# meudnaes/VoronoiRT

Hardware: AMD Instinct MI355X
Metric: formal-solve cell-updates/sec (higher is better)
Workload: dtype f64

## Files before the change

include/voronoirt.h:

```cpp
#ifndef VORONOIRT_H
#define VORONOIRT_H

#include <stdint.h>

#ifdef __cplusplus
extern "C" {
#endif

#define VRT_OK 0
#define VRT_EINVAL (-1)
#define VRT_EGRID (-2)
#define VRT_ENODEVICE (-3)
#define VRT_ENOMEM (-4)
#define VRT_EIO (-5)

typedef struct vrt_grid vrt_grid;
typedef struct vrt_plan vrt_plan;

#define VRT_ALPHA_SITE 0
#define VRT_ALPHA_SITE_LAM 1
#define VRT_ALPHA_ANGLE_SITE_LAM 2
#define VRT_ALPHA_ANGLE_NATIVE 3
#define VRT_ALPHA_SITE_LAM_NATIVE 4

// ... 80 lines not shown
                                     double *max_rel_change, void *stream);
int vrt_rates_populations_native_dev_f32(vrt_plan *p, int64_t nlam, const double *lambda, const int64_t blocks[6],
                                         const float *dJ_up, const float *dJ_down, const double *planck2,
                                         double lambda0, double c0, const double *d_doppler_width, const double *d_gamma,
                                         double sigma_bb_const, const double *sigma_bf1, const double *sigma_bf2,
                                         const double *d_temperature, const double *d_lte_populations, double hc_over_kB,
                                         double pref_ij, double pref_ji, const double *d_C, const double *d_atom_density,
                                         double *d_R, double *d_populations, void *stream);

int vrt_plan_execute_dev_f32(vrt_plan *p, int64_t nlam, int64_t ld, const float *dS,
                             const float *dalpha, int alpha_mode, const float *dI0_up,
                             const float *dI0_down, const double *weights_host, float *dJ,
                             float *dI_out, void *stream);
int vrt_plan_last_sweep_timing(const vrt_plan *p, double *ms, int64_t *launches);
int vrt_plan_patch_layout(const vrt_plan *p, int64_t *out);
int vrt_plan_check(vrt_plan *p);
int vrt_plan_last_path(const vrt_plan *p);
int vrt_plan_set_option(vrt_plan *p, const char *name, const char *value);
int vrt_grid_set_option(vrt_grid *g, const char *name, const char *value);

typedef struct vrt_schedule vrt_schedule;
int vrt_schedule_build(const vrt_grid *g, int dir, const int64_t *up, int n_sweeps, vrt_schedule **out);
int64_t vrt_schedule_num_nodes(const vrt_schedule *s);
int64_t vrt_schedule_num_levels(const vrt_schedule *s);
int vrt_schedule_get(const vrt_schedule *s, int64_t *site, int32_t *zflags, int64_t *level_off);
void vrt_schedule_destroy(vrt_schedule *s);
int vrt_layer_schedule(const vrt_grid *g, int dir, const int64_t *up, int n_sweeps, uint32_t *vis,
                       int32_t *nlev, int64_t *n_visits);
int vrt_layer_sorted_slots(const vrt_grid *g, int dir, const uint32_t *vis, int64_t *store, int64_t *self);

// ... 240 lines not shown
```

voronoirt_amd/_lib.py:

```python
from __future__ import annotations

import ctypes
import os

HERE = os.path.dirname(os.path.abspath(__file__))
LIB_PATH = os.path.join(HERE, "libvrt_hip.so")
if os.environ.get("VRT_LIB_PATH"):
    LIB_PATH = os.environ["VRT_LIB_PATH"]

c_i64 = ctypes.c_int64
c_dbl = ctypes.c_double
p_i64 = ctypes.POINTER(ctypes.c_int64)
p_i32 = ctypes.POINTER(ctypes.c_int32)
p_dbl = ctypes.POINTER(ctypes.c_double)
p_int = ctypes.POINTER(ctypes.c_int)
vp = ctypes.c_void_p

VRT_OK, VRT_EINVAL, VRT_EGRID, VRT_ENODEVICE, VRT_ENOMEM, VRT_EIO = 0, -1, -2, -3, -4, -5
ALPHA_SITE, ALPHA_SITE_LAM, ALPHA_ANGLE_SITE_LAM, ALPHA_ANGLE_NATIVE, ALPHA_SITE_LAM_NATIVE = 0, 1, 2, 3, 4
METRIC_EUCLIDEAN, METRIC_PERIODIC_XY = 0, 1
RASTER_NEAREST, RASTER_INV_DIST2 = 1, 2

class LineCaseStruct(ctypes.Structure):
    _fields_ = [("nlam", c_i64), ("lambda_", p_dbl), ("blocks", c_i64 * 6), ("lambda0", c_dbl), ("c0", c_dbl),
# ... 80 lines not shown
    "vrt_multi_set_shard": (ctypes.c_int, [vp, ctypes.c_char_p]),
    "vrt_multi_last_shard": (ctypes.c_int, [vp]),
    "vrt_multi_uses_rccl": (ctypes.c_int, [vp]),
    "vrt_multi_destroy": (None, [vp]),
    "vrt_multi_execute_line": (ctypes.c_int, [vp, c_i64, c_i64, p_dbl, c_dbl, c_dbl, p_dbl, p_dbl, p_dbl, p_dbl, p_dbl, p_dbl,
                                              p_dbl, p_dbl, p_dbl, p_dbl]),
    "vrt_multi_lambda_create": (ctypes.c_int, [vp, ctypes.POINTER(LineCaseStruct), p_dbl, ctypes.POINTER(vp)]),
    "vrt_multi_lambda_iterate": (ctypes.c_int, [vp, p_dbl]),
    "vrt_multi_lambda_get": (ctypes.c_int, [vp, p_dbl, p_dbl, p_dbl, p_dbl, p_dbl]),
    "vrt_multi_lambda_destroy": (None, [vp]),
    "vrt_rates_populations_dev": (ctypes.c_int, [vp, c_i64, c_i64, p_dbl, p_i64, vp, p_dbl, c_dbl, c_dbl, vp, vp,
                                                 c_dbl, p_dbl, p_dbl, vp, vp, c_dbl, c_dbl, c_dbl, vp, vp, vp,
                                                 vp, vp]),
    "vrt_plan_last_sweep_timing": (ctypes.c_int, [vp, p_dbl, p_i64]),
    "vrt_plan_patch_layout": (ctypes.c_int, [vp, p_i64]),
    "vrt_plan_last_path": (ctypes.c_int, [vp]),
    "vrt_plan_set_option": (ctypes.c_int, [vp, ctypes.c_char_p, ctypes.c_char_p]),
    "vrt_grid_set_option": (ctypes.c_int, [vp, ctypes.c_char_p, ctypes.c_char_p]),
    "vrt_schedule_build": (ctypes.c_int, [vp, ctypes.c_int, p_i64, ctypes.c_int,
                                          ctypes.POINTER(vp)]),
    "vrt_schedule_num_nodes": (c_i64, [vp]),
    "vrt_schedule_num_levels": (c_i64, [vp]),
    "vrt_schedule_get": (ctypes.c_int, [vp, p_i64, p_i32, p_i64]),
    "vrt_schedule_destroy": (None, [vp]),
    "vrt_layer_schedule": (ctypes.c_int, [vp, ctypes.c_int, p_i64, ctypes.c_int,
                                          ctypes.POINTER(ctypes.c_uint32), p_i32, p_i64]),
    "vrt_layer_sorted_slots": (ctypes.c_int, [vp, ctypes.c_int, ctypes.POINTER(ctypes.c_uint32), p_i64, p_i64]),
    "vrt_patch_schedule_build": (ctypes.c_int, [vp, ctypes.c_int, p_i64, ctypes.c_int, ctypes.c_int, ctypes.c_int,
                                                ctypes.POINTER(vp), p_i64]),
    "vrt_patch_schedule_get": (ctypes.c_int, [vp, p_i32, p_i32, p_i32, p_i32, p_i64, p_i32,
# ... 127 lines not shown
```

voronoirt_amd/csrc/vrt_api.cpp:

```cpp
#include <algorithm>
#include <atomic>
#include <chrono>
#include <cmath>
#include <cstdio>
#include <cstdlib>
#include <cstring>
#include <memory>
#include <new>
#include <thread>

#include "vrt_internal.h"

namespace vrt {

static thread_local std::string g_err;

void set_error(const std::string &msg) { g_err = msg; }
int fail(int code, const std::string &msg)
{
    g_err = msg;
    return code;
}

int check_source(const double *S, int64_t count)
// ... 14 lines not shown
{
    if (S)
        if (int rc = check_source(S, n * nlam)) return rc;
    if (populations)
        for (int64_t i = 0; i < 3 * n; i++)
            if (!std::isfinite(populations[i]) || !(populations[i] >= 0.0))
                return fail(VRT_EINVAL, "the populations must be finite and >= 0 everywhere");
    return VRT_OK;
}

void tuning_from_env(Tuning &t)
{
    static const char *names[] = {"VRT_PATH", "VRT_STEP_K", "VRT_STEP_SINGLE", "VRT_STEP_PAIRS", "VRT_STEP_XCD",
                                  "VRT_STEP_STREAMS", "VRT_STEP_LEVEL_MAP", "VRT_STEP_GROUP_DIR", "VRT_TILE_WIDE",
                                  "VRT_TILE_PRE", "VRT_PATCH_K", "VRT_PATCH_NT", "VRT_PATCH_OWN",
                                  "VRT_PATCH_Q", "VRT_PATCH_TARGET", "VRT_PATCH_SPLIT", "VRT_PAIR_BLOCK", "VRT_PATCH_QUAD", "VRT_PATCH_LEAN", "VRT_PATCH_CHAIN", "VRT_CHAIN_PAIRS", "VRT_CHAIN_SPIN", "VRT_CHAIN_DATAFLAG", "VRT_CHAIN_STATIC", "VRT_LAMBDA_NATIVE", "VRT_DEBUG_FLAGS", "VRT_DEBUG_SKIP_LEVELS",
                                  "VRT_TILE_DEBUG"};
    for (const char *nm : names) {
        const char *e = std::getenv(nm);
        if (e && *e && tuning_set(t, nm, e, false) != VRT_OK) {
            static std::mutex mu;
            static std::vector<std::string> said;
            std::lock_guard<std::mutex> lock(mu);
            if (std::find(said.begin(), said.end(), std::string(nm)) == said.end()) {
                said.push_back(nm);
                std::fprintf(stderr, "[libvrt_hip] ignoring %s=%s: %s\n", nm, e, g_err.c_str());
            }
        }
    }
}

// ... 7 lines not shown
            if (v == paths[i]) { t.path = i; return VRT_OK; }
        if (v.empty()) { t.path = 0; return VRT_OK; }
        return fail(VRT_EINVAL, "VRT_PATH must be auto, levels, tiles, steps or patches");
    }
    char *end = nullptr;
    const long x = std::strtol(value, &end, 10);
    if (end == value || *end != 0) return fail(VRT_EINVAL, "option " + nm + " needs an integer value");
    struct { const char *name; int *field; long lo, hi; bool creation_only; } tab[] = {
        {"VRT_STEP_K", &t.step_K, 0, 18, false}, {"VRT_STEP_SINGLE", &t.step_single, 0, 1, false},
        {"VRT_STEP_PAIRS", &t.step_pairs, 0, 64, false}, {"VRT_STEP_XCD", &t.step_xcd, 0, 2, false},
        {"VRT_STEP_STREAMS", &t.step_streams, 1, 4, false}, {"VRT_STEP_LEVEL_MAP", &t.step_level_map, 0, 1, false},
        {"VRT_STEP_GROUP_DIR", &t.step_group_dir, 0, 1, false}, {"VRT_TILE_WIDE", &t.tile_wide, 0, 1, false},
        {"VRT_TILE_PRE", &t.tile_pre, 0, 1, false},
        {"VRT_PATCH_K", &t.patch_K, 1, 8, true}, {"VRT_PATCH_NT", &t.patch_NT, 64, 1024, true},
        {"VRT_PATCH_OWN", &t.patch_own, 0, 65535, true}, {"VRT_PATCH_Q", &t.patch_Q, 1, 4, false},
        {"VRT_PATCH_TARGET", &t.patch_target, 0, 1 << 20, false}, {"VRT_PATCH_SPLIT", &t.patch_split, 0, 4096, false}, {"VRT_PAIR_BLOCK", &t.pair_block, 1, 16, true},
        {"VRT_PATCH_QUAD", &t.patch_quad, 0, 1, true}, {"VRT_PATCH_LEAN", &t.patch_lean, 0, 1, false},
        {"VRT_PATCH_CHAIN", &t.patch_chain, 0, 2, false}, {"VRT_CHAIN_PAIRS", &t.chain_pairs, 1, 256, false},
        {"VRT_CHAIN_SPIN", &t.chain_spin, 1, 1 << 20, false}, {"VRT_CHAIN_DATAFLAG", &t.chain_dataflag, 0, 2, false},
        {"VRT_LAMBDA_NATIVE", &t.lambda_native, 0, 1, false}, {"VRT_CHAIN_STATIC", &t.chain_static, 0, 1, false}, {"VRT_DEBUG_FLAGS", &t.debug_flags, 0, 1 << 20, false},
        {"VRT_DEBUG_SKIP_LEVELS", &t.debug_skip_levels, 0, 1, false}, {"VRT_TILE_DEBUG", &t.tile_debug, 0, 1, false},
    };
    for (auto &o : tab)
        if (nm == o.name) {
            if (o.creation_only && created)
                return fail(VRT_EINVAL, "option " + nm + " shapes what plan creation builds: preset it in the environment");
            if (x < o.lo || x > o.hi) return fail(VRT_EINVAL, "option " + nm + " out of range");
            *o.field = (int)x;
            return VRT_OK;
        }
    return fail(VRT_EINVAL, "unknown option " + nm);
// ... 1185 lines not shown
        fewest = INT64_MAX;
        for (int a = 0; a < p->A; a++)
            for (int layer = 2; layer <= maxL; layer++) {
                const int32_t *first = p->h_patch_first.data() + (size_t)a * (size_t)(maxL + 2);
                fewest = std::min<int64_t>(fewest, first[layer + 1] - first[layer]);
            }
        if (fewest == INT64_MAX) fewest = 0;
    }
    out[0] = p->patch_ok ? p->n_patches : 0;
    out[1] = fewest;
    out[2] = p->patch_work_off.empty() ? 0 : p->patch_work_off.back();
    out[3] = p->patch_work_padding;
    return VRT_OK;
}

int vrt_plan_last_sweep_timing(const vrt_plan *p, double *ms, int64_t *launches)
{
    if (!p) return fail(VRT_EINVAL, "NULL plan");
    if (!p->ev_valid) return fail(VRT_EINVAL, "no execute has run on this plan yet");
    return guarded([&] {
        VRT_HIP_TRY(hipEventSynchronize(p->ev1));
        float t = 0.f;
        VRT_HIP_TRY(hipEventElapsedTime(&t, p->ev0, p->ev1));
        if (ms) *ms = (double)t;
        if (launches) *launches = p->last_launches;
        return patch_chain_check(const_cast<vrt_plan *>(p));
    });
}

int vrt_plan_last_path(const vrt_plan *p) { return p ? p->last_path : 0; }
// ... 302 lines not shown
```

voronoirt_amd/csrc/vrt_internal.h:

```cpp
#pragma once

#include <hip/hip_runtime.h>

#include <algorithm>
#include <cstdint>
#include <memory>
#include <mutex>
#include <new>
#include <string>
#include <thread>
#include <vector>

#include "voronoirt.h"

namespace vrt {

void set_error(const std::string &msg);
int fail(int code, const std::string &msg);

int check_source(const double *S, int64_t count);
int check_state_pointers(const void *session, const double *S, const double *populations);
int check_state(int64_t n, int64_t nlam, const double *S, const double *populations);

#define VRT_HIP_TRY(expr)                                                                  \
// ... 211 lines not shown
    int step_group_dir = 1;
    int tile_wide = 1;
    int tile_pre = 1;
    int patch_K = 1, patch_NT = 512;
    int patch_own = 0;
    int patch_Q = 1;
    int pair_block = 1;
    int patch_quad = 1;
    int patch_lean = 1;
    int patch_chain = 2;
    int chain_pairs = 9;
    int chain_spin = 2048;
    int chain_dataflag = 2;
    int patch_split = 0;
    int patch_target = 0;
    int chain_static = 1;
    int lambda_native = 1;
    int debug_flags = 0, debug_skip_levels = 0, tile_debug = 0;
};
void tuning_from_env(Tuning &t);
int tuning_set(Tuning &t, const char *name, const char *value, bool created);

struct ExecArgs {
    int64_t nlam = 0, ld = 0;
    const void *S = nullptr;
    const void *S_nat[2] = {nullptr, nullptr};
    const void *alpha = nullptr;
    int alpha_mode = 0;
    const void *I0[2] = {nullptr, nullptr};
    const double *weights = nullptr;
// ... 153 lines not shown
    int chain_npair = -1, chain_lgB = -1, chain_nsplit = -1, chain_reduce = -1;
    int64_t chain_items = 0;
    struct ChainSet {
        int npair = -1, lgB = -1, nsplit = -1, reduce = -1;
        vrt::DevBuf<int4> items;
        vrt::DevBuf<int32_t> deps;
        int q_off[9] = {0, 0, 0, 0, 0, 0, 0, 0, 0};
        int64_t n_items = 0;
    };
    std::vector<ChainSet> chain_cache;
    uint32_t chain_epoch = 0;
    vrt::DevBuf<int4> d_patch_work;
    std::vector<int64_t> patch_work_off;
    int patch_work_groups = 0;
    int64_t patch_work_padding = 0;
    vrt::Stream step_stream[4];
    vrt::Event step_fork, step_join[4];
    int last_path = 0;
    vrt::Event ev0, ev1;
    bool ev_valid = false;
    std::vector<vrt::CopyLane> copy_lanes;
    vrt::Event copy_done;
    int64_t last_launches = 0;
    std::mutex mu;
};

namespace vrt {

struct PlanDelete { void operator()(vrt_plan *p) const { vrt_plan_destroy(p); } };
using PlanPtr = std::unique_ptr<vrt_plan, PlanDelete>;
// ... 136 lines not shown
int plane_from_native_f32(vrt_plan *p, int dir_index, int64_t nlam, int64_t ld, const float *din, float *dout, hipStream_t st);
int J_from_native_f32(vrt_plan *p, int64_t nlam, int64_t ld, const float *dJ_up, const float *dJ_down, float *dJ, hipStream_t st);
int planes_to_native(vrt_plan *p, int64_t nlam, int64_t ld, const double *din, double *out_up, double *out_down, hipStream_t st);
int plane_from_native(vrt_plan *p, int dir_index, int64_t nlam, int64_t ld, const double *din, double *dout, hipStream_t st);
int J_from_native(vrt_plan *p, int64_t nlam, int64_t ld, const double *dJ_up, const double *dJ_down, double *dJ, hipStream_t st);
int execute_layers(vrt_plan *p, const ExecArgs &x, int path);
int64_t steps_max_layer(bool f32);

struct TileArgs;
struct PatchReduce;
bool patch_shape_exists(int K, int Q, int NT);
int launch_patch_entries(vrt_plan *p, int a, int64_t first, int64_t count);
int ensure_patch_work(vrt_plan *p, int G, const std::vector<int32_t> &group_angles, const std::vector<int> &group_off);
int launch_patch_layer(vrt_plan *p, const TileArgs &ta, int npair, int layer, int group, int Q, hipStream_t st,
                       bool f32, const PatchReduce *reduce);
bool patch_chain_possible(const vrt_plan *p, int npair, bool f32);
bool patch_chain_dataflag(const vrt_plan *p, int npair, bool f32);
int launch_patch_chain(vrt_plan *p, const TileArgs &ta, int npair, hipStream_t st, bool f32, const PatchReduce *reduce,
                       bool dataflag, bool ctrl_zeroed = false);
int chain_ctrl_words();
int patch_chain_check(vrt_plan *p);

struct NgRange {
    int64_t dense = 0, tail = 0, tstride = 1;
};
struct NgState {
    int order = 0, start = 0, period = 0;
    DevBuf<double> hist[3];
    unsigned have = 0;
    DevBuf<double> d_ws;
// ... 12 lines not shown
```

voronoirt_amd/csrc/vrt_layers.hip:

```cpp
#include <hip/hip_runtime.h>

#include <algorithm>
#include <cmath>
#include <cstdio>
#include <cstdlib>
#include <cstring>

#include "vrt_device.h"
#include "vrt_internal.h"

#include "vrt_layout_kernels.h"
#include "vrt_step_kernels.h"
#include "vrt_tile_kernels.h"

namespace vrt {

static int build_task_map(vrt_plan *p, int nlam, hipStream_t st)
{
    const int A = p->A;
    if (p->task_map_nlam == nlam && p->d_task_map) return VRT_OK;
    const int ntask = A * nlam;
    struct Group { int a, l0, l1; double cost; };
    std::vector<Group> groups;
    const int halves = nlam >= 2 ? 2 : 1;
// ... 649 lines not shown
            if (upto <= reduced_upto[d]) continue;
            red.lo[k] = (int)reduced_upto[d];
            red.hi[k] = (int)upto;
            red.Jd[k] = J_planes(p, x, d);
            red.count[k] = 0;
            for (int a = 0; a < A; a++)
                if ((p->dir_of_active[(size_t)a] > 0) == (d == 0)) red.angles[k][red.count[k]++] = a;
            reduced_upto[d] = upto;
            k++;
        }
        return k > 0;
    };
    const int Lmax = deepest_layer(r);
    if ((rc = fork_streams(p, st, G))) return rc;
    r.launches = 0;
    for (int layer = 2; layer <= Lmax; layer++)
        for (int gi = 0; gi < G; gi++) {
            hipStream_t sg = gi == 0 ? st : p->step_stream[gi];
            if (p->step_group_off[gi + 1] == p->step_group_off[gi]) continue;
            int Q = p->tune.patch_Q;
            if (!patch_shape_exists(p->patch_K, Q, p->patch_NT) || (npair % Q != 0 && npair < 2 * Q)) Q = 1;
            PatchReduce red;
            const bool have_red = make_reduce(gi, layer - 1, false, red);
            if ((rc = launch_patch_layer(p, r.ta, npair, layer, gi, Q, sg, kF32, have_red ? &red : nullptr))) return rc;
            r.launches += 1;
        }
    for (int gi = 0; gi < G; gi++) {
        PatchReduce red;
        if (!make_reduce(gi, 0, true, red)) continue;
        if ((rc = launch_patch_layer(p, r.ta, npair, p->tile_max_layers + 1, gi, 1, gi == 0 ? st : p->step_stream[gi], kF32, &red)))
// ... 139 lines not shown
```

voronoirt_amd/csrc/vrt_patch.hip:

```cpp
#include <hip/hip_runtime.h>

#include <algorithm>
#include <cmath>
#include <cstdio>
#include <cstdlib>
#include <cstring>
#include <type_traits>

#include "vrt_device.h"
#include "vrt_internal.h"

namespace vrt {

enum : int {
    kDiagNoLevels = 1, kDiagCentreGathers = 2, kDiagNoWeights = 4, kDiagNoStores = 8, kDiagNoGatherI = 16, kDiagNoGatherAlpha = 32,
    kDiagNoGatherS = 64, kDiagNoReduce = 128, kDiagNoWait = 256, kDiagPlainLoadI = 512, kDiagPlainStoreI = 1024, kDiagNoPairLoop = 2048,
    kDiagDirectTable = 4096,
};
__host__ __device__ __forceinline__ constexpr bool diag(int dbg, int flag) { return kDiag && (dbg & flag) != 0; }

struct PatchArgs {
    TileArgs ta;
    int npair;
    int layer;
    int ngrp;
    int nrow;
    int nsplit, Q;
    int sbase, srem;
    int lgB;
    int stride;
    int cap;
    int quad;
    int lean;
    int dbg_ent0, dbg_ent_stride, dbg_ent_last;
    int dbg;
    PatchReduce red;
    const int4 *wrec;
    const int32_t *e_pos, *e_u1, *e_u2;
    const uint32_t *e_vis, *e_loc;
    const double *e_w1, *e_w2, *e_r1, *e_r2;
};

__global__ void __launch_bounds__(256)
k_patch_entries(int64_t count, const int32_t *__restrict__ e_pos, const int32_t *__restrict__ t_u1,
                const int32_t *__restrict__ t_u2, const double *__restrict__ t_w1, const double *__restrict__ t_w2,
                const double *__restrict__ t_r1, const double *__restrict__ t_r2, int32_t *__restrict__ e_u1,
                int32_t *__restrict__ e_u2, double *__restrict__ e_w1, double *__restrict__ e_w2,
                double *__restrict__ e_r1, double *__restrict__ e_r2)
{
    const int64_t e = (int64_t)blockIdx.x * blockDim.x + threadIdx.x;
// ... 32 lines not shown
    const int nstep = (nblock + pa.Q - 1) / pa.Q;
    pa.sbase = nstep / pa.nsplit;
    pa.srem = nstep - pa.sbase * pa.nsplit;
}
__host__ __device__ __forceinline__ void split_blocks(const PatchArgs &pa, int split, int nblock, int &b0, int &b1)
{
    const int base = pa.sbase, rem = pa.srem;
    const int s0 = split * base + (split < rem ? split : rem), s1 = s0 + base + (split < rem ? 1 : 0);
    b0 = s0 * pa.Q;
    b1 = nblock < s1 * pa.Q ? nblock : s1 * pa.Q;
}

#ifndef VRT_REDUCE_LAST
#define VRT_REDUCE_LAST 1
#endif
__device__ __forceinline__ int reduce_block_index(const PatchArgs &pa)
{
    const int rows = (int)gridDim.y - pa.nrow;
    const int y = VRT_REDUCE_LAST ? (int)blockIdx.y - pa.nrow : ((int)blockIdx.y < rows ? (int)blockIdx.y : -1);
    return y < 0 ? -1 : y * (int)gridDim.x + (int)blockIdx.x;
}
__device__ __forceinline__ int patch_row(const PatchArgs &pa)
{
    return VRT_REDUCE_LAST ? (int)blockIdx.y : (int)blockIdx.y - ((int)gridDim.y - pa.nrow);
}
template <typename T, int NT>
__device__ __forceinline__ void patch_reduce_role(const PatchArgs &pa)
{
    typedef typename Pair<T>::type T2;
    const TileArgs &ta = pa.ta;
    const int tid = threadIdx.x;
    int b = reduce_block_index(pa), r = 0;
    if (b >= pa.red.nblk[0]) { b -= pa.red.nblk[0]; r = 1; }
    if (b >= pa.red.nblk[r]) return;
    if (diag(pa.dbg, kDiagNoReduce)) return;
    const int len = pa.red.hi[r] - pa.red.lo[r];
    const int per = NT * pa.red.ppb;
    const int nblock = pair_block_count(pa.npair, pa.lgB);
    int k0 = 0, lw = 0;
    for (int k = 0; k < nblock; k++) {
// ... 48 lines not shown
}

#ifdef VRT_PATCH_WPE
#define VRT_WPE_ATTR __attribute__((amdgpu_waves_per_eu(VRT_PATCH_WPE, VRT_PATCH_WPE)))
#else
#define VRT_WPE_ATTR
#endif
template <typename T, int AM, int K, int Q, int NT>
__global__ void __launch_bounds__(NT) VRT_WPE_ATTR
k_patch_solve(PatchArgs pa)
{
    typedef typename Pair<T>::type T2;
    extern __shared__ __attribute__((aligned(16))) double2 ptile[];
    const TileArgs &ta = pa.ta;
    const int tid = threadIdx.x;
    if (reduce_block_index(pa) >= 0) {
        patch_reduce_role<T, NT>(pa);
        return;
    }
    const int x = (int)blockIdx.x & 7, grp = (int)blockIdx.x >> 3, sj = patch_row(pa);
    const int4 rec = pa.wrec[2 * (sj * 8 + x)], rec2 = pa.wrec[2 * (sj * 8 + x) + 1];
    if (rec.y <= 0) return;
    const int sib = grp & ((1 << pa.lgB) - 1);
    const int nblock = pair_block_count(pa.npair, pa.lgB);
    int b0, b1;
    split_blocks(pa, grp >> pa.lgB, nblock, b0, b1);
    if (b0 >= b1) return;
    {
        int k0, lw;
        pair_block_of(b0, pa.npair, pa.lgB, k0, lw);
        if (sib >= (1 << lw)) return;
    }
    const int ent_off = rec.x, n_ent = rec.y, own_lo = rec.z, own_cnt = rec.w;
    const int dbg = kDiag ? pa.dbg : 0;
    const int nlev = diag(dbg, kDiagNoLevels) ? 0 : rec2.x, a = rec2.y & 0xFFFF;
    const int d = rec2.y >> 16;
    const int lo = rec2.z, hi = rec2.w;
    const int64_t n = ta.n;
    const int stride = pa.stride;

    double *s_w1 = reinterpret_cast<double *>(ptile + Q * stride);
    double *s_w2 = s_w1 + pa.cap, *s_r1 = s_w2 + pa.cap, *s_r2 = s_r1 + pa.cap;
    int *s_pos = reinterpret_cast<int *>(s_r2 + pa.cap);
    int *s_u1 = s_pos + pa.cap, *s_u2 = s_u1 + pa.cap;
    uint32_t *s_vis = reinterpret_cast<uint32_t *>(s_u2 + pa.cap), *s_loc = s_vis + pa.cap;
#pragma unroll
    for (int k = 0; k < K; k++) {
// ... 119 lines not shown
            }
        }
    }
}


typedef int vrt_i32x8 __attribute__((ext_vector_type(8)));
typedef const __attribute__((address_space(4))) vrt_i32x8 WorkRec;
static_assert(2 * sizeof(int4) == 32 && sizeof(vrt_i32x8) == 32, "a work-list slot is two int4: 32 bytes, 32-byte aligned");
struct PatchItem {
    int sib, b0, b1;
    int ent_off, n_ent, own_lo, own_cnt, nlev, a, d, lo, hi;
};
__device__ __forceinline__ bool patch_item(const PatchArgs &pa, int lgS, PatchItem &it)
{
    const int x = (int)blockIdx.x & 7, grp = (int)blockIdx.x >> 3, sj = patch_row(pa);
    const vrt_i32x8 r8 = *((const WorkRec *)(uintptr_t)pa.wrec + (sj * 8 + x));
    const int4 rec = make_int4(r8[0], r8[1], r8[2], r8[3]), rec2 = make_int4(r8[4], r8[5], r8[6], r8[7]);
    if (rec.y <= 0) return false;
    it.sib = grp & ((1 << lgS) - 1);
    split_blocks(pa, grp >> lgS, pair_block_count(pa.npair, pa.lgB), it.b0, it.b1);
    if (it.b0 >= it.b1) return false;
    it.ent_off = rec.x; it.n_ent = rec.y; it.own_lo = rec.z; it.own_cnt = rec.w;
    it.nlev = rec2.x; it.a = rec2.y & 0xFFFF;
    it.d = rec2.y >> 16;
    it.lo = rec2.z;
    it.hi = rec2.w;
    return true;
}
template <int CAP>
struct EntryTable {
    double *w1, *w2, *r1, *r2;
    int *pos, *u1, *u2;
    uint32_t *vis, *loc;
    __device__ __forceinline__ EntryTable(double2 *tiles, int planes)
    {
// ... 378 lines not shown
            } else {
                T2 *I = reinterpret_cast<T2 *>(pa.I) + (size_t)it.a * pa.npair * (size_t)n + qb;
                *reinterpret_cast<T2 *>(reinterpret_cast<char *>(I) + ((unsigned)(it.own_lo + tid) << sh)) = from_d2<T>(ptile[tid]);
            }
        }
        __syncthreads();
    }
}

template <typename T, int AM, int NT>
__global__ void __launch_bounds__(NT) VRT_LEAN_ATTR
k_patch_lean(PatchArgs pa)
{
    extern __shared__ __attribute__((aligned(16))) double2 ptile[];
    const int tid = threadIdx.x;
    if (reduce_block_index(pa) >= 0) {
        patch_reduce_role<T, NT>(pa);
        return;
    }
    const double e2 = exp2_table_load();
    typename EntryTable<NT>::Regs early{};
    if (diag(pa.dbg, kDiagDirectTable))
        early = EntryTable<NT>::load(pa, min(pa.dbg_ent0 + (patch_row(pa) * 8 + ((int)blockIdx.x & 7)) * pa.dbg_ent_stride + tid, pa.dbg_ent_last));
    PatchItem it;
    if (!patch_item(pa, pa.lgB, it)) return;
    if (diag(pa.dbg, kDiagNoPairLoop)) it.b1 = it.b0;
    const EntryTable<NT> tab(ptile, 1);
    if (tid == 0) ptile[it.n_ent] = make_double2(0.0, 0.0);
    if (diag(pa.dbg, kDiagDirectTable)) tab.store(early, it, tid);
    else tab.park(pa, it, tid);
    exp2_table_store(e2);
    __syncthreads();
    lean_pairs<T, AM, NT, 0>(pair_io<AM>(pa, it.d), it, tab, ptile);
}


template <int AM, int NT, bool CHAIN>
__device__ __forceinline__ void quad_pairs(const PairIO &pa, const PatchItem &it, const EntryTable<NT> &tab,
                                           double2 *ptile)
{
// ... 109 lines not shown
            }
        }
        __syncthreads();
    }
}

#ifndef VRT_QUAD_ATTR
#define VRT_QUAD_ATTR __attribute__((amdgpu_waves_per_eu(6, 6)))
#endif
template <int AM, int NT>
__global__ void __launch_bounds__(NT) VRT_QUAD_ATTR
k_patch_quad(PatchArgs pa)
{
    extern __shared__ __attribute__((aligned(16))) double2 ptile[];
    const int tid = threadIdx.x;
    if (reduce_block_index(pa) >= 0) {
        patch_reduce_role<float, NT>(pa);
        return;
    }
    const double e2 = exp2_table_load();
    PatchItem it;
    if (!patch_item(pa, pa.lgB - 1, it)) return;
    const EntryTable<NT> tab(ptile, 2);
    if (tid == 0) {
        ptile[it.n_ent] = make_double2(0.0, 0.0);
        ptile[NT + 1 + it.n_ent] = make_double2(0.0, 0.0);
    }
    tab.park(pa, it, tid);
    exp2_table_store(e2);
    __syncthreads();
    quad_pairs<AM, NT, false>(pair_io<AM>(pa, it.d), it, tab, ptile);
}


struct ChainDev {
    TileArgs ta;
    int npair, nsplit, cap;
// ... 388 lines not shown
            const int s_min = (int)std::min<int64_t>(steps_all, std::max<int64_t>(1, (512 + items - 1) / items));
            double dmin = 1e300;
            for (int c = steps_all; c >= 1; c--) {
                const int sc = (steps_all + c - 1) / c;
                if (sc >= s_min) dmin = std::min(dmin, std::fabs(std::log((double)items * sc / T)));
            }
            nsplit = s_min;
            for (int c = steps_all; c >= 1; c--) {
                const int sc = (steps_all + c - 1) / c;
                if (sc >= s_min && std::fabs(std::log((double)items * sc / T)) <= dmin + 0.03) nsplit = sc;
            }
        }
        pa.nsplit = nsplit;
        pa.ngrp = nsplit << lgS;
    }
    set_split(pa, pair_block_count(npair, pa.lgB));
    pa.stride = p->patch_cap + 1;
    pa.cap = p->patch_cap;
    pa.dbg = kDiag ? p->tune.debug_flags : 0;
    {
        const int64_t slots = std::max<int64_t>(1, p->patch_work_off.back());
        pa.dbg_ent_stride = (int)std::max<int64_t>(1, p->n_patch_entries / slots);
        pa.dbg_ent0 = (int)(w0 * pa.dbg_ent_stride);
        pa.dbg_ent_last = (int)std::max<int64_t>(0, p->n_patch_entries - 1);
    }
    pa.wrec = p->d_patch_work + 2 * w0;
    pa.e_pos = p->e_pos; pa.e_u1 = p->e_u1; pa.e_u2 = p->e_u2;
    pa.e_vis = p->e_vis; pa.e_loc = p->e_loc;
    pa.e_w1 = p->e_w1; pa.e_w2 = p->e_w2; pa.e_r1 = p->e_r1; pa.e_r2 = p->e_r2;
    pa.nrow = (int)((w1 - w0) / 8);
    int64_t gx = 8 * (int64_t)pa.ngrp;
    if (pa.nrow == 0) gx = std::max<int64_t>(gx, (((int64_t)pa.red.nred + 65534) / 65535 + 7) / 8 * 8);
    const int64_t gy = pa.nrow + (pa.red.nred + gx - 1) / gx;
    if (gy > 65535 || gx > INT32_MAX)
        return fail(VRT_EINVAL, "a layer of this size needs more than 65535 rows of patch and reduction blocks in one launch");
    const dim3 grid((unsigned)gx, (unsigned)gy);
    const size_t lds = (size_t)(pa.quad ? 2 : Q) * (size_t)pa.stride * sizeof(double2) + (size_t)pa.cap * (4 * sizeof(double) + 5 * sizeof(int32_t));
    const int rc = f32 ? launch_mode<float>(ta.alpha_mode, p->patch_K, Q, p->patch_NT, grid, lds, st, pa)
                       : launch_mode<double>(ta.alpha_mode, p->patch_K, Q, p->patch_NT, grid, lds, st, pa);
    return rc;
}

bool patch_chain_possible(const vrt_plan *p, int npair, bool f32)
{
    if (!p->patch_ok || p->tune.patch_chain == 0 || p->patch_K != 1 || p->patch_NT != 512) return false;
    const int lgB = native_lg(p, f32);
    const bool quad = f32 && lgB >= 1 && p->tune.patch_quad != 0 && (npair & 1) == 0;
    if (lgB - (quad ? 1 : 0) != 0) return false;
    if (!f32 && p->tune.patch_lean == 0) return false;
    if (p->tile_max_layers >= 65535 || p->A > 63) return false;
    if (p->tune.patch_chain == 1) return true;
    if (f32) return false;
    const double per_layer = (double)p->n_patches / (double)std::max(1, p->tile_max_layers);
    return per_layer * (double)pair_block_count(npair, lgB) <= 1400.0;
}
// ... 296 lines not shown
```

Before: 89.46 billion.

## Reorder patch-layer grid so split index maps to grid rows, add diagnostic timeline

```diff
diff --git a/include/voronoirt.h b/include/voronoirt.h
--- a/include/voronoirt.h
+++ b/include/voronoirt.h
@@ -118,6 +118,8 @@
                              float *dI_out, void *stream);
 int vrt_plan_last_sweep_timing(const vrt_plan *p, double *ms, int64_t *launches);
 int vrt_plan_patch_layout(const vrt_plan *p, int64_t *out);
+int vrt_patch_dispatch_map(int order, int nrow, int nsplit, int lg_siblings, int64_t nred, int steps, int64_t *dims, int32_t *blocks);
+int vrt_plan_patch_timeline(vrt_plan *p, int64_t cap_launches, int64_t cap_blocks, int64_t *launches, uint64_t *stamps, int64_t *counts);
 int vrt_plan_check(vrt_plan *p);
 int vrt_plan_last_path(const vrt_plan *p);
 int vrt_plan_set_option(vrt_plan *p, const char *name, const char *value);
diff --git a/voronoirt_amd/_lib.py b/voronoirt_amd/_lib.py
--- a/voronoirt_amd/_lib.py
+++ b/voronoirt_amd/_lib.py
@@ -118,6 +118,8 @@
                                                  vp, vp]),
     "vrt_plan_last_sweep_timing": (ctypes.c_int, [vp, p_dbl, p_i64]),
     "vrt_plan_patch_layout": (ctypes.c_int, [vp, p_i64]),
+    "vrt_patch_dispatch_map": (ctypes.c_int, [ctypes.c_int, ctypes.c_int, ctypes.c_int, ctypes.c_int, c_i64, ctypes.c_int, p_i64, p_i32]),
+    "vrt_plan_patch_timeline": (ctypes.c_int, [vp, c_i64, c_i64, p_i64, ctypes.POINTER(ctypes.c_uint64), p_i64]),
     "vrt_plan_last_path": (ctypes.c_int, [vp]),
     "vrt_plan_set_option": (ctypes.c_int, [vp, ctypes.c_char_p, ctypes.c_char_p]),
     "vrt_grid_set_option": (ctypes.c_int, [vp, ctypes.c_char_p, ctypes.c_char_p]),
diff --git a/voronoirt_amd/csrc/vrt_api.cpp b/voronoirt_amd/csrc/vrt_api.cpp
--- a/voronoirt_amd/csrc/vrt_api.cpp
+++ b/voronoirt_amd/csrc/vrt_api.cpp
@@ -52,7 +52,7 @@
     static const char *names[] = {"VRT_PATH", "VRT_STEP_K", "VRT_STEP_SINGLE", "VRT_STEP_PAIRS", "VRT_STEP_XCD",
                                   "VRT_STEP_STREAMS", "VRT_STEP_LEVEL_MAP", "VRT_STEP_GROUP_DIR", "VRT_TILE_WIDE",
                                   "VRT_TILE_PRE", "VRT_PATCH_K", "VRT_PATCH_NT", "VRT_PATCH_OWN",
-                                  "VRT_PATCH_Q", "VRT_PATCH_TARGET", "VRT_PATCH_SPLIT", "VRT_PAIR_BLOCK", "VRT_PATCH_QUAD", "VRT_PATCH_LEAN", "VRT_PATCH_CHAIN", "VRT_CHAIN_PAIRS", "VRT_CHAIN_SPIN", "VRT_CHAIN_DATAFLAG", "VRT_CHAIN_STATIC", "VRT_LAMBDA_NATIVE", "VRT_DEBUG_FLAGS", "VRT_DEBUG_SKIP_LEVELS",
+                                  "VRT_PATCH_Q", "VRT_PATCH_TARGET", "VRT_PATCH_SPLIT", "VRT_PATCH_ORDER", "VRT_PATCH_TIMELINE", "VRT_PAIR_BLOCK", "VRT_PATCH_QUAD", "VRT_PATCH_LEAN", "VRT_PATCH_CHAIN", "VRT_CHAIN_PAIRS", "VRT_CHAIN_SPIN", "VRT_CHAIN_DATAFLAG", "VRT_CHAIN_STATIC", "VRT_LAMBDA_NATIVE", "VRT_DEBUG_FLAGS", "VRT_DEBUG_SKIP_LEVELS",
                                   "VRT_TILE_DEBUG"};
     for (const char *nm : names) {
         const char *e = std::getenv(nm);
@@ -90,7 +90,8 @@
         {"VRT_TILE_PRE", &t.tile_pre, 0, 1, false},
         {"VRT_PATCH_K", &t.patch_K, 1, 8, true}, {"VRT_PATCH_NT", &t.patch_NT, 64, 1024, true},
         {"VRT_PATCH_OWN", &t.patch_own, 0, 65535, true}, {"VRT_PATCH_Q", &t.patch_Q, 1, 4, false},
-        {"VRT_PATCH_TARGET", &t.patch_target, 0, 1 << 20, false}, {"VRT_PATCH_SPLIT", &t.patch_split, 0, 4096, false}, {"VRT_PAIR_BLOCK", &t.pair_block, 1, 16, true},
+        {"VRT_PATCH_TARGET", &t.patch_target, 0, 1 << 20, false}, {"VRT_PATCH_SPLIT", &t.patch_split, 0, 4096, false}, {"VRT_PATCH_ORDER", &t.patch_order, 0, 1, false},
+        {"VRT_PATCH_TIMELINE", &t.patch_timeline, 0, 1, false}, {"VRT_PAIR_BLOCK", &t.pair_block, 1, 16, true},
         {"VRT_PATCH_QUAD", &t.patch_quad, 0, 1, true}, {"VRT_PATCH_LEAN", &t.patch_lean, 0, 1, false},
         {"VRT_PATCH_CHAIN", &t.patch_chain, 0, 2, false}, {"VRT_CHAIN_PAIRS", &t.chain_pairs, 1, 256, false},
         {"VRT_CHAIN_SPIN", &t.chain_spin, 1, 1 << 20, false}, {"VRT_CHAIN_DATAFLAG", &t.chain_dataflag, 0, 2, false},
@@ -1306,6 +1307,21 @@
     return VRT_OK;
 }
 
+int vrt_patch_dispatch_map(int order, int nrow, int nsplit, int lg_siblings, int64_t nred, int steps, int64_t *dims, int32_t *blocks)
+{
+    return guarded([&] { return patch_dispatch_map(order, nrow, nsplit, lg_siblings, nred, steps, dims, blocks); });
+}
+
+int vrt_plan_patch_timeline(vrt_plan *p, int64_t cap_launches, int64_t cap_blocks, int64_t *launches, uint64_t *stamps, int64_t *counts)
+{
+    if (!p || !launches || !stamps || !counts) return fail(VRT_EINVAL, "NULL plan or output");
+    return guarded([&] {
+        std::lock_guard<std::mutex> lock(p->mu);
+        if (int rc = use_device(p->device)) return rc;
+        return patch_timeline_read(p, cap_launches, cap_blocks, launches, stamps, counts);
+    });
+}
+
 int vrt_plan_last_sweep_timing(const vrt_plan *p, double *ms, int64_t *launches)
 {
     if (!p) return fail(VRT_EINVAL, "NULL plan");
diff --git a/voronoirt_amd/csrc/vrt_internal.h b/voronoirt_amd/csrc/vrt_internal.h
--- a/voronoirt_amd/csrc/vrt_internal.h
+++ b/voronoirt_amd/csrc/vrt_internal.h
@@ -249,6 +249,8 @@
     int chain_dataflag = 2;
     int patch_split = 0;
     int patch_target = 0;
+    int patch_order = 1;
+    int patch_timeline = 0;
     int chain_static = 1;
     int lambda_native = 1;
     int debug_flags = 0, debug_skip_levels = 0, tile_debug = 0;
@@ -432,6 +434,9 @@
     std::vector<int64_t> patch_work_off;
     int patch_work_groups = 0;
     int64_t patch_work_padding = 0;
+    vrt::DevBuf<unsigned long long> d_patch_tl;
+    std::vector<int64_t> patch_tl_launches;
+    int64_t patch_tl_blocks = 0;
     vrt::Stream step_stream[4];
     vrt::Event step_fork, step_join[4];
     int last_path = 0;
@@ -598,6 +603,10 @@
 int ensure_patch_work(vrt_plan *p, int G, const std::vector<int32_t> &group_angles, const std::vector<int> &group_off);
 int launch_patch_layer(vrt_plan *p, const TileArgs &ta, int npair, int layer, int group, int Q, hipStream_t st,
                        bool f32, const PatchReduce *reduce);
+constexpr int kPatchTimelineRec = 12;
+void patch_timeline_begin(vrt_plan *p);
+int patch_timeline_read(vrt_plan *p, int64_t cap_launches, int64_t cap_blocks, int64_t *launches, uint64_t *stamps, int64_t *counts);
+int patch_dispatch_map(int order, int nrow, int nsplit, int lg_siblings, int64_t nred, int steps, int64_t *dims, int32_t *blocks);
 bool patch_chain_possible(const vrt_plan *p, int npair, bool f32);
 bool patch_chain_dataflag(const vrt_plan *p, int npair, bool f32);
 int launch_patch_chain(vrt_plan *p, const TileArgs &ta, int npair, hipStream_t st, bool f32, const PatchReduce *reduce,
diff --git a/voronoirt_amd/csrc/vrt_layers.hip b/voronoirt_amd/csrc/vrt_layers.hip
--- a/voronoirt_amd/csrc/vrt_layers.hip
+++ b/voronoirt_amd/csrc/vrt_layers.hip
@@ -687,6 +687,7 @@
     const int Lmax = deepest_layer(r);
     if ((rc = fork_streams(p, st, G))) return rc;
     r.launches = 0;
+    if (kDiag) patch_timeline_begin(p);
     for (int layer = 2; layer <= Lmax; layer++)
         for (int gi = 0; gi < G; gi++) {
             hipStream_t sg = gi == 0 ? st : p->step_stream[gi];
diff --git a/voronoirt_amd/csrc/vrt_patch.hip b/voronoirt_amd/csrc/vrt_patch.hip
--- a/voronoirt_amd/csrc/vrt_patch.hip
+++ b/voronoirt_amd/csrc/vrt_patch.hip
@@ -25,6 +25,9 @@
     int layer;
     int ngrp;
     int nrow;
+    int order;
+    int prow;
+    unsigned row_rcp;
     int nsplit, Q;
     int sbase, srem;
     int lgB;
@@ -34,6 +37,7 @@
     int lean;
     int dbg_ent0, dbg_ent_stride, dbg_ent_last;
     int dbg;
+    unsigned long long *tl;
     PatchReduce red;
     const int4 *wrec;
     const int32_t *e_pos, *e_u1, *e_u2;
@@ -96,16 +100,88 @@
 #ifndef VRT_REDUCE_LAST
 #define VRT_REDUCE_LAST 1
 #endif
+struct PatchBlock { int lane, row, split, sib; };
+__host__ __device__ __forceinline__ PatchBlock patch_block_of(int order, int nrow, unsigned row_rcp, int lgS, unsigned bx, unsigned y)
+{
+    PatchBlock b;
+    const int grp = (int)(bx >> 3);
+    b.lane = (int)(bx & 7u);
+    if (order == 0) {
+        b.row = (int)y;
+        b.split = grp >> lgS;
+        b.sib = grp & ((1 << lgS) - 1);
+    } else {
+        b.split = (int)(((unsigned long long)(2u * y) * row_rcp) >> 32);
+        b.row = (int)y - b.split * nrow;
+        b.sib = grp;
+    }
+    return b;
+}
+struct PatchGrid {
+    int order = 0, prow = 0;
+    unsigned row_rcp = 0;
+    int64_t gx = 0, gy = 0;
+};
+static PatchGrid patch_grid(int order, int nrow, int nsplit, int lgS, int64_t nred)
+{
+    PatchGrid g;
+    if (order == 1 && nsplit >= 2 && nrow >= 1) {
+        g.gx = (int64_t)8 << lgS;
+        g.prow = nsplit * nrow;
+        g.gy = (int64_t)nsplit * nrow + (nred + g.gx - 1) / g.gx;
+        if (g.gy <= 65535) {
+            g.order = 1;
+            g.row_rcp = (unsigned)((((uint64_t)1 << 31) + (uint64_t)nrow - 1) / (uint64_t)nrow);
+            return g;
+        }
+    }
+    g.order = 0;
+    g.prow = nrow;
+    g.row_rcp = 0;
+    g.gx = (int64_t)8 * ((int64_t)nsplit << lgS);
+    if (nrow == 0) g.gx = std::max<int64_t>(g.gx, ((nred + 65534) / 65535 + 7) / 8 * 8);
+    g.gy = nrow + (nred + g.gx - 1) / g.gx;
+    return g;
+}
 __device__ __forceinline__ int reduce_block_index(const PatchArgs &pa)
 {
-    const int rows = (int)gridDim.y - pa.nrow;
-    const int y = VRT_REDUCE_LAST ? (int)blockIdx.y - pa.nrow : ((int)blockIdx.y < rows ? (int)blockIdx.y : -1);
+    const int rows = (int)gridDim.y - pa.prow;
+    const int y = VRT_REDUCE_LAST ? (int)blockIdx.y - pa.prow : ((int)blockIdx.y < rows ? (int)blockIdx.y : -1);
     return y < 0 ? -1 : y * (int)gridDim.x + (int)blockIdx.x;
 }
-__device__ __forceinline__ int patch_row(const PatchArgs &pa)
-{
-    return VRT_REDUCE_LAST ? (int)blockIdx.y : (int)blockIdx.y - ((int)gridDim.y - pa.nrow);
-}
+__device__ __forceinline__ PatchBlock patch_block(const PatchArgs &pa, int lgS)
+{
+    const int y = VRT_REDUCE_LAST ? (int)blockIdx.y : (int)blockIdx.y - ((int)gridDim.y - pa.prow);
+    return patch_block_of(pa.order, pa.nrow, pa.row_rcp, lgS, blockIdx.x, (unsigned)y);
+}
+__device__ __forceinline__ int patch_row(const PatchArgs &pa) { return patch_block(pa, 0).row; }
+struct BlockStamp {
+    unsigned long long *slot = nullptr;
+    unsigned long long t0 = 0, share = 0;
+    __device__ __forceinline__ explicit BlockStamp(const PatchArgs &pa)
+    {
+        if (kDiag && pa.tl) {
+            slot = pa.tl + 3 * ((size_t)blockIdx.y * gridDim.x + blockIdx.x);
+            t0 = wall_clock64();
+        }
+    }
+    __device__ __forceinline__ void steps(const PatchArgs &pa, int b0, int b1)
+    {
+        if (kDiag) share = (unsigned long long)((b1 - b0 + pa.Q - 1) / pa.Q);
+    }
+    __device__ __forceinline__ void reduces()
+    {
+        if (kDiag) share = 1ull << 32;
+    }
+    __device__ __forceinline__ ~BlockStamp()
+    {
+        if (kDiag && slot && threadIdx.x == 0) {
+            slot[0] = t0;
+            slot[1] = wall_clock64();
+            slot[2] = share;
+        }
+    }
+};
 template <typename T, int NT>
 __device__ __forceinline__ void patch_reduce_role(const PatchArgs &pa)
 {
@@ -184,23 +260,27 @@
     extern __shared__ __attribute__((aligned(16))) double2 ptile[];
     const TileArgs &ta = pa.ta;
     const int tid = threadIdx.x;
+    BlockStamp stamp(pa);
     if (reduce_block_index(pa) >= 0) {
+        stamp.reduces();
         patch_reduce_role<T, NT>(pa);
         return;
     }
-    const int x = (int)blockIdx.x & 7, grp = (int)blockIdx.x >> 3, sj = patch_row(pa);
+    const PatchBlock blk = patch_block(pa, pa.lgB);
+    const int x = blk.lane, sj = blk.row;
     const int4 rec = pa.wrec[2 * (sj * 8 + x)], rec2 = pa.wrec[2 * (sj * 8 + x) + 1];
     if (rec.y <= 0) return;
-    const int sib = grp & ((1 << pa.lgB) - 1);
+    const int sib = blk.sib;
     const int nblock = pair_block_count(pa.npair, pa.lgB);
     int b0, b1;
-    split_blocks(pa, grp >> pa.lgB, nblock, b0, b1);
+    split_blocks(pa, blk.split, nblock, b0, b1);
     if (b0 >= b1) return;
     {
         int k0, lw;
         pair_block_of(b0, pa.npair, pa.lgB, k0, lw);
         if (sib >= (1 << lw)) return;
     }
+    stamp.steps(pa, b0, b1);
     const int ent_off = rec.x, n_ent = rec.y, own_lo = rec.z, own_cnt = rec.w;
     const int dbg = kDiag ? pa.dbg : 0;
     const int nlev = diag(dbg, kDiagNoLevels) ? 0 : rec2.x, a = rec2.y & 0xFFFF;
@@ -350,12 +430,13 @@
 };
 __device__ __forceinline__ bool patch_item(const PatchArgs &pa, int lgS, PatchItem &it)
 {
-    const int x = (int)blockIdx.x & 7, grp = (int)blockIdx.x >> 3, sj = patch_row(pa);
+    const PatchBlock blk = patch_block(pa, lgS);
+    const int x = blk.lane, sj = blk.row;
     const vrt_i32x8 r8 = *((const WorkRec *)(uintptr_t)pa.wrec + (sj * 8 + x));
     const int4 rec = make_int4(r8[0], r8[1], r8[2], r8[3]), rec2 = make_int4(r8[4], r8[5], r8[6], r8[7]);
     if (rec.y <= 0) return false;
-    it.sib = grp & ((1 << lgS) - 1);
-    split_blocks(pa, grp >> lgS, pair_block_count(pa.npair, pa.lgB), it.b0, it.b1);
+    it.sib = blk.sib;
+    split_blocks(pa, blk.split, pair_block_count(pa.npair, pa.lgB), it.b0, it.b1);
     if (it.b0 >= it.b1) return false;
     it.ent_off = rec.x; it.n_ent = rec.y; it.own_lo = rec.z; it.own_cnt = rec.w;
     it.nlev = rec2.x; it.a = rec2.y & 0xFFFF;
@@ -764,7 +845,9 @@
 {
     extern __shared__ __attribute__((aligned(16))) double2 ptile[];
     const int tid = threadIdx.x;
+    BlockStamp stamp(pa);
     if (reduce_block_index(pa) >= 0) {
+        stamp.reduces();
         patch_reduce_role<T, NT>(pa);
         return;
     }
@@ -774,6 +857,7 @@
         early = EntryTable<NT>::load(pa, min(pa.dbg_ent0 + (patch_row(pa) * 8 + ((int)blockIdx.x & 7)) * pa.dbg_ent_stride + tid, pa.dbg_ent_last));
     PatchItem it;
     if (!patch_item(pa, pa.lgB, it)) return;
+    stamp.steps(pa, it.b0, it.b1);
     if (diag(pa.dbg, kDiagNoPairLoop)) it.b1 = it.b0;
     const EntryTable<NT> tab(ptile, 1);
     if (tid == 0) ptile[it.n_ent] = make_double2(0.0, 0.0);
@@ -913,13 +997,16 @@
 {
     extern __shared__ __attribute__((aligned(16))) double2 ptile[];
     const int tid = threadIdx.x;
+    BlockStamp stamp(pa);
     if (reduce_block_index(pa) >= 0) {
+        stamp.reduces();
         patch_reduce_role<float, NT>(pa);
         return;
     }
     const double e2 = exp2_table_load();
     PatchItem it;
     if (!patch_item(pa, pa.lgB - 1, it)) return;
+    stamp.steps(pa, it.b0, it.b1);
     const EntryTable<NT> tab(ptile, 2);
     if (tid == 0) {
         ptile[it.n_ent] = make_double2(0.0, 0.0);
@@ -1338,7 +1425,6 @@
         pa.nsplit = nsplit;
         pa.ngrp = nsplit << lgS;
     }
-    set_split(pa, pair_block_count(npair, pa.lgB));
     pa.stride = p->patch_cap + 1;
     pa.cap = p->patch_cap;
     pa.dbg = kDiag ? p->tune.debug_flags : 0;
@@ -1353,16 +1439,82 @@
     pa.e_vis = p->e_vis; pa.e_loc = p->e_loc;
     pa.e_w1 = p->e_w1; pa.e_w2 = p->e_w2; pa.e_r1 = p->e_r1; pa.e_r2 = p->e_r2;
     pa.nrow = (int)((w1 - w0) / 8);
-    int64_t gx = 8 * (int64_t)pa.ngrp;
-    if (pa.nrow == 0) gx = std::max<int64_t>(gx, (((int64_t)pa.red.nred + 65534) / 65535 + 7) / 8 * 8);
-    const int64_t gy = pa.nrow + (pa.red.nred + gx - 1) / gx;
+    const PatchGrid pg = patch_grid(p->tune.patch_order, pa.nrow, pa.nsplit, lgS, pa.red.nred);
+    pa.order = pg.order;
+    pa.prow = pg.prow;
+    pa.row_rcp = pg.row_rcp;
+    set_split(pa, pair_block_count(npair, pa.lgB));
+    const int64_t gx = pg.gx, gy = pg.gy;
     if (gy > 65535 || gx > INT32_MAX)
         return fail(VRT_EINVAL, "a layer of this size needs more than 65535 rows of patch and reduction blocks in one launch");
+    pa.tl = nullptr;
+    if (kDiag && p->tune.patch_timeline) {
+        const int64_t cap = (int64_t)1 << 20, blocks = gx * gy;
+        if (!p->d_patch_tl && p->d_patch_tl.alloc((size_t)(3 * cap)) != VRT_OK) return VRT_ENOMEM;
+        if (p->patch_tl_blocks + blocks <= cap) {
+            pa.tl = p->d_patch_tl + 3 * p->patch_tl_blocks;
+            const int64_t rec[kPatchTimelineRec] = {layer, group, gx, gy, pa.nrow, pa.nsplit, lgS, pa.order, pa.prow, pa.red.nred,
+                                                    p->patch_tl_blocks, (pair_block_count(npair, pa.lgB) + Q - 1) / Q};
+            p->patch_tl_launches.insert(p->patch_tl_launches.end(), rec, rec + kPatchTimelineRec);
+            p->patch_tl_blocks += blocks;
+        }
+    }
     const dim3 grid((unsigned)gx, (unsigned)gy);
     const size_t lds = (size_t)(pa.quad ? 2 : Q) * (size_t)pa.stride * sizeof(double2) + (size_t)pa.cap * (4 * sizeof(double) + 5 * sizeof(int32_t));
     const int rc = f32 ? launch_mode<float>(ta.alpha_mode, p->patch_K, Q, p->patch_NT, grid, lds, st, pa)
                        : launch_mode<double>(ta.alpha_mode, p->patch_K, Q, p->patch_NT, grid, lds, st, pa);
     return rc;
+}
+
+void patch_timeline_begin(vrt_plan *p)
+{
+    p->patch_tl_launches.clear();
+    p->patch_tl_blocks = 0;
+}
+
+int patch_timeline_read(vrt_plan *p, int64_t cap_launches, int64_t cap_blocks, int64_t *launches, uint64_t *stamps, int64_t *counts)
+{
+    if (!kDiag) return fail(VRT_EINVAL, "the timeline of the patch launches exists in the -DVRT_DIAG build only");
+    const int64_t nl = (int64_t)p->patch_tl_launches.size() / kPatchTimelineRec, nb = p->patch_tl_blocks;
+    if (nl > cap_launches || nb > cap_blocks) return fail(VRT_EINVAL, "timeline buffers too small");
+    VRT_HIP_TRY(hipDeviceSynchronize());
+    int khz = 0;
+    VRT_HIP_TRY(hipDeviceGetAttribute(&khz, hipDeviceAttributeWallClockRate, p->device));
+    counts[0] = nl; counts[1] = nb; counts[2] = khz;
+    std::copy(p->patch_tl_launches.begin(), p->patch_tl_launches.end(), launches);
+    if (nb > 0) VRT_HIP_TRY(hipMemcpy(stamps, p->d_patch_tl, sizeof(uint64_t) * 3 * (size_t)nb, hipMemcpyDeviceToHost));
+    return VRT_OK;
+}
+
+int patch_dispatch_map(int order, int nrow, int nsplit, int lg_siblings, int64_t nred, int steps, int64_t *dims, int32_t *blocks)
+{
+    if (!dims) return fail(VRT_EINVAL, "NULL output");
+    if (order < 0 || order > 1 || nrow < 0 || nrow > 65535 || nsplit < 1 || nsplit > 4096 || lg_siblings < 0 || lg_siblings > 4 ||
+        nred < 0 || nred > INT32_MAX || steps < nsplit)
+        return fail(VRT_EINVAL, "dispatch map: argument out of range");
+    const PatchGrid pg = patch_grid(order, nrow, nsplit, lg_siblings, nred);
+    if (pg.gy > 65535) return fail(VRT_EINVAL, "more than 65535 rows of patch and reduction blocks");
+    dims[0] = pg.gx; dims[1] = pg.gy; dims[2] = pg.order; dims[3] = pg.prow;
+    if (!blocks) return VRT_OK;
+    PatchArgs sp;
+    sp.nsplit = nsplit;
+    sp.Q = 1;
+    set_split(sp, steps);
+    for (int64_t by = 0; by < pg.gy; by++)
+        for (int64_t bx = 0; bx < pg.gx; bx++) {
+            int32_t *o = blocks + 6 * (by * pg.gx + bx);
+            std::fill(o, o + 6, 0);
+            if (by >= pg.prow) {
+                o[0] = 1;
+                o[1] = (int32_t)((by - pg.prow) * pg.gx + bx);
+                continue;
+            }
+            const PatchBlock b = patch_block_of(pg.order, nrow, pg.row_rcp, lg_siblings, (unsigned)bx, (unsigned)by);
+            int b0, b1;
+            split_blocks(sp, b.split, steps, b0, b1);
+            o[1] = b.lane; o[2] = b.row; o[3] = b.split; o[4] = b.sib; o[5] = b1 - b0;
+        }
+    return VRT_OK;
 }
 
 bool patch_chain_possible(const vrt_plan *p, int npair, bool f32)
```

After: 91.16 billion, median of 6. 1.9% higher.
